# enricobottazzi/zk-fhe

Measured on AMD Instinct MI355X. Metric: BFV proofs/sec (k=13), higher is better.
Workload: dtype u32x8 (256-bit Montgomery integers over BN254 Fr/Fq)

## Files before the change

### include/zkfhe.h

```cpp
#ifndef ZKFHE_H
#define ZKFHE_H
#include <stddef.h>
#include <stdint.h>

#ifdef __cplusplus
extern "C" {
#endif

#define ZKFHE_OK 0
#define ZKFHE_EINVAL (-1)
#define ZKFHE_EHIP (-2)
#define ZKFHE_ENOMEM (-3)
#define ZKFHE_ENODEV (-4)

typedef struct zkfhe_ctx zkfhe_ctx;
typedef struct zkfhe_basis zkfhe_basis;

typedef struct { uint64_t l[4]; } zkfhe_fr;
typedef struct { uint64_t l[4]; } zkfhe_fq;
typedef struct { zkfhe_fq x, y; } zkfhe_g1_affine;
typedef struct { zkfhe_fq x, y, zz, zzz; } zkfhe_g1_xyzz;

int zkfhe_ctx_create(int device_id, void *hip_stream, zkfhe_ctx **out);
int zkfhe_ctx_destroy(zkfhe_ctx *ctx);
// ... 140 lines not shown

typedef struct zkfhe_srs zkfhe_srs;
#define ZKFHE_SRS_HALO2_UNSAFE "halo2:ParamsKZG::setup(k, ChaCha20Rng::from_seed([0u8; 32]))"
int zkfhe_srs_create(zkfhe_ctx *ctx, uint32_t k, const uint8_t *seed, size_t seed_len, zkfhe_srs **out);
int zkfhe_srs_save(zkfhe_ctx *ctx, const zkfhe_srs *srs, const char *path);
int zkfhe_srs_drop_host_copy(zkfhe_srs *srs);
int zkfhe_srs_load(zkfhe_ctx *ctx, const char *path, zkfhe_srs **out);
int zkfhe_srs_g2(const zkfhe_srs *srs, uint8_t g2_le[128], uint8_t s_g2_le[128]);
int zkfhe_srs_set_g2(zkfhe_srs *srs, const uint8_t g2_le[128], const uint8_t s_g2_le[128]);
int zkfhe_srs_file_g2(const char *path, uint32_t *k_out, uint8_t g2_le[128], uint8_t s_g2_le[128]);
int zkfhe_chacha20_block(const uint8_t key[32], const uint32_t counter_nonce[4], uint8_t out[64]);
int zkfhe_srs_from_points(zkfhe_ctx *ctx, uint32_t k, const zkfhe_g1_affine *g_host, const zkfhe_g1_affine *g_lagrange_host, zkfhe_srs **out);
int zkfhe_srs_create_sharded(zkfhe_ctx *ctx, zkfhe_comm *comm, uint32_t k, const uint8_t *seed, size_t seed_len, zkfhe_srs **out);
int zkfhe_srs_destroy(zkfhe_ctx *ctx, zkfhe_srs *srs);
int zkfhe_srs_table_bits(const zkfhe_srs *srs, int *wide_calls);
int zkfhe_srs_table_info(const zkfhe_srs *srs, int bits[2], uint64_t *bytes, int *narrowed);

typedef struct zkfhe_bfv_pk zkfhe_bfv_pk;
int zkfhe_bfv_keygen(zkfhe_ctx *ctx, const zkfhe_srs *srs, const char *input_json, const zkfhe_bfv_params *params,
                     const zkfhe_bfv_config *config, zkfhe_bfv_pk **out);
int zkfhe_bfv_pk_destroy(zkfhe_ctx *ctx, zkfhe_bfv_pk *pk);
int zkfhe_bfv_pk_release_ctx(zkfhe_ctx *ctx, zkfhe_bfv_pk *pk);
int zkfhe_bfv_pk_info(const zkfhe_bfv_pk *pk, uint8_t vk_digest[32], uint32_t *n_fixed, uint32_t *n_sigma);
int zkfhe_bfv_pk_commitments(const zkfhe_bfv_pk *pk, uint8_t *fixed_out, uint8_t *sigma_out);
int zkfhe_bfv_pk_prefix_cache(const zkfhe_bfv_pk *pk, int capacity, uint64_t *hits, uint64_t *misses, uint64_t *entries);
int zkfhe_bfv_pk_prehash(const zkfhe_bfv_pk *pk, const char *input_json, uint64_t *started, uint64_t *taken, uint64_t *pending);
int zkfhe_bfv_pk_break_points(const zkfhe_bfv_pk *pk, int which, uint32_t *out, uint32_t *count);

int zkfhe_bfv_pk_export_vk(const zkfhe_bfv_pk *pk, uint8_t *out, size_t cap, size_t *len);
int zkfhe_bfv_witness_stream(zkfhe_ctx *ctx, const zkfhe_bfv_pk *pk, const char *input_json, const uint8_t gamma_le[32], uint8_t *cells_out,
                             size_t cap_cells, size_t *n_cells);
int zkfhe_lookup_permute(zkfhe_ctx *ctx, const zkfhe_fr *cols_dev, size_t n_cols, size_t n, uint32_t usable_rows, zkfhe_fr *a_dev,
                         zkfhe_fr *s_dev, int *not_in_table);
int zkfhe_bfv_pk_save(zkfhe_ctx *ctx, const zkfhe_bfv_pk *pk, const char *path);
int zkfhe_bfv_pk_load(zkfhe_ctx *ctx, const zkfhe_srs *srs, const char *path, zkfhe_bfv_pk **out);

int zkfhe_snark_encode(const uint8_t *instances_le, size_t n_instances, const uint8_t *proof, size_t proof_len, uint8_t *out, size_t cap, size_t *len);
int zkfhe_snark_decode(const uint8_t *snark, size_t snark_len, uint8_t *instances_le, size_t *n_instances, uint8_t *proof, size_t *proof_len);

int zkfhe_bfv_verify(const uint8_t *vk_bytes, size_t vk_len, const uint8_t *instances, size_t n_instances, const uint8_t *proof,
                     size_t proof_len, const uint8_t *srs_seed, size_t seed_len, int *accepted, char *err, size_t err_len);
int zkfhe_bfv_verify_g2(const uint8_t *vk_bytes, size_t vk_len, const uint8_t *instances, size_t n_instances, const uint8_t *proof, size_t proof_len,
                        const uint8_t g2[128], const uint8_t s_g2[128], int *accepted, char *err, size_t err_len);

int zkfhe_bfv_verify_batch(zkfhe_ctx *ctx, const uint8_t *vk_bytes, size_t vk_len, size_t n_proofs, const uint8_t *const *instances,
                           const size_t *n_instances, const uint8_t *const *proofs, const size_t *proof_lens, const uint8_t *srs_seed,
                           size_t seed_len, const uint8_t *g2, const uint8_t *s_g2, int *accepted, char *errs, size_t err_stride);

int zkfhe_bfv_prove(zkfhe_ctx *ctx, const zkfhe_srs *srs, const zkfhe_bfv_pk *pk, const char *input_json,
                    const uint8_t seed[32], uint8_t *proof_out, size_t proof_cap, size_t *proof_len,
                    uint8_t *instances_out, size_t *n_instances, float *timings_ms);

typedef struct {
  const uint64_t *pk0, *pk1, *m, *u, *e0, *e1, *c0, *c1;
} zkfhe_bfv_words;
int zkfhe_bfv_prove_words(zkfhe_ctx *ctx, const zkfhe_srs *srs, const zkfhe_bfv_pk *pk, const zkfhe_bfv_words *in, const uint8_t seed[32],
                          uint8_t *proof_out, size_t proof_cap, size_t *proof_len, uint8_t *instances_out, size_t *n_instances, float *timings_ms);

int zkfhe_poly_mul_ternary_negacyclic(zkfhe_ctx *ctx, const uint64_t *a_dev, size_t a_count, const uint64_t *s_dev, size_t n_polys,
                                      uint64_t n, uint64_t q, uint64_t *out_dev, int *not_ternary);
int zkfhe_bfv_error_cdt(const zkfhe_bfv_params *params, uint64_t *thresholds, size_t *count);
int zkfhe_bfv_fhe_keypair(zkfhe_ctx *ctx, const zkfhe_bfv_params *params, const uint8_t seed[32], uint64_t *sk_out, uint64_t *pk0_out,
                          uint64_t *pk1_out);
int zkfhe_bfv_encrypt(zkfhe_ctx *ctx, const zkfhe_bfv_params *params, const uint64_t *pk0, const uint64_t *pk1, size_t n_msgs,
                      const uint64_t *m, const uint8_t seed[32], uint64_t first_index, uint64_t *u_out, uint64_t *e0_out,
                      uint64_t *e1_out, uint64_t *c0_out, uint64_t *c1_out);
// ... 73 lines not shown
```

### zk-fhe_amd/__init__.py

```python
import ctypes
import os

import numpy as np

_HERE = os.path.dirname(os.path.abspath(__file__))
LIB_PATH = os.path.join(_HERE, "libzkfhe_hip.so")
_lib = None

PROF_G1_DECOMPRESS, PROF_MSM_SEGMENTED = 3, 4
PROF_BFV_SAMPLE, PROF_RNS_NTT, PROF_RNS_EPILOGUE = 5, 6, 7
PROF_BFV_TENSOR, PROF_BFV_RELIN, PROF_BFV_EVAL_EPILOGUE, PROF_BFV_ELEMENTWISE = 8, 9, 10, 11
PROF_BFV_SHARE_SUM, PROF_BFV_DECRYPT_COMBINE = 12, 13
PROF_BFV_GALOIS, PROF_BFV_SLOT_NTT = 14, 15
PROF_BFV_HOIST, PROF_BFV_LINEAR = 16, 17

EXPORTS = [
    "zkfhe_ctx_create", "zkfhe_ctx_destroy", "zkfhe_last_error", "zkfhe_sync", "zkfhe_stream", "zkfhe_device_info",
    "zkfhe_dev_alloc", "zkfhe_dev_free", "zkfhe_upload", "zkfhe_download", "zkfhe_copy_dev", "zkfhe_memset_dev",
    "zkfhe_timer_start", "zkfhe_timer_stop_ms", "zkfhe_prof_enable", "zkfhe_prof_reset", "zkfhe_prof_read", "zkfhe_prof_read_ops", "zkfhe_ctx_last_proof_marks",
    "zkfhe_fr_add", "zkfhe_fr_sub", "zkfhe_fr_mul", "zkfhe_fr_scale", "zkfhe_fr_to_mont", "zkfhe_fr_from_mont",
    "zkfhe_fr_batch_invert", "zkfhe_fr_sqr_chain", "zkfhe_fq29_sqr_chain",
    "zkfhe_ntt_batch", "zkfhe_ntt_batch_to", "zkfhe_coset_ntt_batch",
    "zkfhe_basis_create", "zkfhe_basis_destroy", "zkfhe_basis_len", "zkfhe_msm_batch",
    "zkfhe_g1_add", "zkfhe_g1_mul", "zkfhe_msm_sparse", "zkfhe_msm_batch_xyzz", "zkfhe_msm_sparse_xyzz", "zkfhe_g1_xyzz_to_affine", "zkfhe_basis_has_multiples", "zkfhe_basis_table_bits", "zkfhe_basis_table_bytes", "zkfhe_srs_table_bits", "zkfhe_srs_table_info",
    "zkfhe_comm_unique_id", "zkfhe_comm_create", "zkfhe_comm_create_with_transport", "zkfhe_comm_destroy", "zkfhe_comm_rank", "zkfhe_comm_world", "zkfhe_comm_active",
    "zkfhe_comm_point_range", "zkfhe_comm_all_gather", "zkfhe_comm_all_gather_async", "zkfhe_msm_batch_sharded", "zkfhe_msm_batch_sharded_async", "zkfhe_comm_join", "zkfhe_comm_record_event", "zkfhe_srs_create_sharded",
    "zkfhe_witness_poly_mul_u64", "zkfhe_host_poly_mul_u32", "zkfhe_witness_div_mod",
    "zkfhe_bfv_build_tables", "zkfhe_bfv_auto_config", "zkfhe_bfv_tables_free", "zkfhe_bfv_tables_count", "zkfhe_bfv_tables_copy_advice",
    "zkfhe_bfv_tables_copy_fixed", "zkfhe_bfv_tables_copy_instance", "zkfhe_bfv_tables_copy_copies",
    "zkfhe_bfv_tables_copy_break_points", "zkfhe_bfv_mock_check", "zkfhe_bfv_tables_poke_advice",
    "zkfhe_srs_create", "zkfhe_srs_from_points", "zkfhe_srs_destroy", "zkfhe_srs_save", "zkfhe_srs_drop_host_copy", "zkfhe_srs_load", "zkfhe_srs_g2", "zkfhe_srs_set_g2", "zkfhe_srs_file_g2",
    "zkfhe_chacha20_block", "zkfhe_snark_encode", "zkfhe_snark_decode", "zkfhe_bfv_keygen", "zkfhe_bfv_pk_destroy", "zkfhe_bfv_pk_release_ctx", "zkfhe_bfv_pk_info", "zkfhe_bfv_pk_prefix_cache",
    "zkfhe_bfv_pk_commitments", "zkfhe_bfv_pk_break_points", "zkfhe_bfv_pk_prehash", "zkfhe_bfv_prove", "zkfhe_bfv_pk_export_vk", "zkfhe_bfv_pk_save", "zkfhe_bfv_pk_load", "zkfhe_bfv_witness_stream", "zkfhe_lookup_permute", "zkfhe_bfv_verify", "zkfhe_bfv_verify_g2",
    "zkfhe_g1_decompress", "zkfhe_msm_segmented", "zkfhe_bfv_verify_batch",
    "zkfhe_poly_mul_ternary_negacyclic", "zkfhe_bfv_error_cdt", "zkfhe_bfv_fhe_keypair", "zkfhe_bfv_encrypt", "zkfhe_bfv_decrypt", "zkfhe_bfv_prove_words",
    "zkfhe_bfv_add", "zkfhe_bfv_sum", "zkfhe_bfv_add_plain", "zkfhe_bfv_mul_plain", "zkfhe_bfv_relin_digits", "zkfhe_bfv_relin_keygen",
    "zkfhe_bfv_mul", "zkfhe_bfv_noise",
    "zkfhe_bfv_keygen_share", "zkfhe_bfv_share_aggregate", "zkfhe_bfv_relin_share1", "zkfhe_bfv_relin_share2", "zkfhe_bfv_decrypt_share",
    "zkfhe_bfv_decrypt_combine",
    "zkfhe_bfv_slot_count", "zkfhe_bfv_galois_element", "zkfhe_bfv_slot_sum_elements", "zkfhe_bfv_encode_slots", "zkfhe_bfv_decode_slots",
    "zkfhe_bfv_galois_keygen", "zkfhe_bfv_apply_galois", "zkfhe_bfv_slot_sum", "zkfhe_bfv_galois_share",
    "zkfhe_bfv_apply_galois_many", "zkfhe_bfv_linear_transform",
    "zkfhe_transcript_create", "zkfhe_transcript_destroy", "zkfhe_transcript_common_scalar", "zkfhe_transcript_write_scalar",
    "zkfhe_transcript_common_point", "zkfhe_transcript_write_point", "zkfhe_transcript_squeeze", "zkfhe_transcript_bytes",
    "zkfhe_poseidon_permute", "zkfhe_poseidon_constants", "zkfhe_poseidon_hash_many", "zkfhe_host_hash_mode", "zkfhe_prover_gate",
    "zkfhe_version",
]


os.environ.setdefault("GPU_MAX_HW_QUEUES", "2")


class ZkfheError(RuntimeError):
    pass


def load_library():
    global _lib
    if _lib is not None:
        return _lib
    if not os.path.exists(LIB_PATH):
        raise ZkfheError("HIP extension %s is missing: run `python zk-fhe_amd/build.py` (or __graft_entry__.build())" % LIB_PATH)
    lib = ctypes.CDLL(LIB_PATH)
    vp, sz, ci = ctypes.c_void_p, ctypes.c_size_t, ctypes.c_int
    lib.zkfhe_last_error.restype = ctypes.c_char_p
    lib.zkfhe_last_error.argtypes = [vp]
# ... 1440 lines not shown
```

### zk-fhe_amd/host/prove.hip

```cpp
#include "prover_internal.hpp"

int alloc_witness_buffers(zkfhe_ctx *ctx, const zkfhe_bfv_pk *pk, Workspace *ws) {
  if (ws->stream.p) return ZKFHE_OK;
  const size_t N = pk->prm.N;
  CK(ws->stream.alloc(ctx, (pk->gate1_cells + 8) * 32));
  CK(ws->pool.alloc(ctx, 40 * (2 * N + 8) * 32));
  CK(ws->invtmp.alloc(ctx, (pk->n_inv_slots + 8) * 32));
  ZK_HIP(ctx, hipHostMalloc((void **)&ws->host_pool, 24 * (2 * N + 8) * 32, hipHostMallocDefault));
  ws->host_poly_len = 2 * N + 8;
  ZK_HIP(ctx, hipHostMalloc((void **)&ws->host_poly, ws->host_poly_len * 32, hipHostMallocDefault));
  CK(ws->wblind.alloc(ctx, 256));
  ZK_HIP(ctx, hipHostMalloc((void **)&ws->ring, Workspace::RING_BYTES, hipHostMallocDefault));
  CK(ws->dev_ring.alloc(ctx, Workspace::RING_BYTES));
  {
    const CircuitConfig &c = pk->cfg;
    const size_t max_items = (size_t)c.n_advice() + c.n_fixed() + 2 + c.n_perm() + c.n_chunks() + 3 * c.n_lookup;
    ws->out_pts_cap = std::max<size_t>(ws->n_all, c.n_perm()) + 16;
    ws->out_ev_off = ws->out_pts_cap * PT_SLOT;
    ws->out_ev_cap = max_items * 4;
    ws->out_flag_off = ws->out_ev_off + ws->out_ev_cap * 32;
    ZK_HIP(ctx, hipHostMalloc((void **)&ws->host_out, ws->out_flag_off + 256, hipHostMallocDefault));
    memset(ws->host_out, 0, ws->out_flag_off + 256);
  }
  ZK_HIP(ctx, hipHostMalloc((void **)&ws->host_pts, ((size_t)pk->cfg.n_gate0 + 1) * PT_SLOT, hipHostMallocDefault));
// ... 433 lines not shown
  std::mutex mu;
  std::condition_variable cv;
  int slots = 0;
  uint64_t next_ticket = 0, serving = 0;
};
struct GateHold {
  bool held = false;
  void enter() { held = HeavyGate::get().enter(); }
  void leave() {
    if (held) HeavyGate::get().leave();
    held = false;
  }
  ~GateHold() { leave(); }
};

struct Trace {
  bool on;
  double t0, last, cpu_last;
  unsigned long tid;
  static double thread_cpu_ms() {
    timespec ts;
    clock_gettime(CLOCK_THREAD_CPUTIME_ID, &ts);
    return ts.tv_sec * 1e3 + ts.tv_nsec * 1e-6;
  }
  Trace() : on(getenv("ZKFHE_TRACE") != nullptr), t0(now_ms()), last(t0), cpu_last(on ? thread_cpu_ms() : 0), tid((unsigned long)std::hash<std::thread::id>()(std::this_thread::get_id()) % 10000) {}
  void mark(const char *what) {
    if (!on) return;
    const double t = now_ms(), c = thread_cpu_ms();
    fprintf(stderr, "[zkfhe trace %04lu] %8.3f ms (+%7.3f, cpu %6.3f) %s @%.3f\n", tid, t - t0, t - last, c - cpu_last, what, t);
    last = t;
    cpu_last = c;
  }
};

int prove_impl(zkfhe_ctx *ctx, const zkfhe_srs *srs, zkfhe_bfv_pk *pk, const char *input_json, const FastInput *words, const uint8_t seed[32],
               std::vector<uint8_t> &proof, std::vector<U256> &instances, float *timings) {
  const CircuitConfig &cfg = pk->cfg;
  const size_t n = cfg.n(), u = cfg.u(), ne = 4 * n;
  const unsigned k = cfg.k;
  const double t_start = now_ms();
  Trace trace;
  zkp::RngSeed rseed;
  memcpy(rseed.w, seed, 32);
  const size_t nbl_all = n - u;
  const uint64_t ctr_adv = 0, ctr_lk = (uint64_t)cfg.n_advice() * nbl_all, ctr_pz = ctr_lk + 2 * (uint64_t)cfg.n_lookup * nbl_all,
                 ctr_lz = ctr_pz + (uint64_t)cfg.n_chunks() * (nbl_all - 1), ctr_rand = ctr_lz + (uint64_t)cfg.n_lookup * (nbl_all - 1);
  auto rng_fill = [&](hipStream_t stream, uint64_t ctr0, uint64_t ctr_col_stride, Fr *dst, size_t per_col, size_t col_stride, size_t n_cols) -> int {
    if (!per_col || !n_cols) return ZKFHE_OK;
    zkp::k_rng_fill<<<grid_for(ctx, per_col * n_cols), 256, 0, stream>>>(rseed, ctr0, ctr_col_stride, dst, per_col, col_stride, n_cols);
    ZK_LAUNCH_CHECK(ctx);
    return ZKFHE_OK;
  };
  Transcript tr(cfg.transcript);
  const NttDomain *dom;
  CK(zk_domain(ctx, (int)k, &dom));
  Workspace *ws;
  CK(get_workspace(ctx, pk, &ws));
  GpuPolyMul gpu_mul(ctx, ws);
  struct BackendGuard {
    explicit BackendGuard(PolyMulBackend *b) { poly_mul_backend() = b; }
    ~BackendGuard() { poly_mul_backend() = nullptr; }
  } guard(&gpu_mul);
  const zkfhe_basis *small_basis = srs->g_lagrange_small ? srs->g_lagrange_small : srs->g_lagrange;
  CK(zkfhe_sync(ctx));
  CK(alloc_witness_buffers(ctx, pk, ws));
  ws->ring_off = ws->ring_flushed = 0;
// ... 229 lines not shown
  const Fr beta = mont(beta_c), gamma = mont(gamma_c);
  GateHold gate;
  if (!srs->sharded()) gate.enter();
  {
    if (instances.size() < ws->inst_count)
      ZK_HIP(ctx, hipMemsetAsync(ws->inst_l.fr() + instances.size(), 0, (ws->inst_count - instances.size()) * 32, ctx->stream));
    if (inst_via_ring) {
      CK(flush_staged(ctx, ws));
      if (!instances.empty()) CK(zkfhe_fr_to_mont(ctx, (const zkfhe_fr *)inst_staged, (zkfhe_fr *)ws->inst_l.p, instances.size()));
    } else {
      CK(upload_canon(ctx, ws->inst_l.fr(), instances.data(), instances.size()));
    }
    ws->inst_count = instances.size();
  }
  U256 dcan;
  memcpy(dcan.l, DELTA_CANON, 32);
  Fr *beta_delta_dev = (Fr *)ws->small.p;
  zkp::k_powers<<<1, 256, 0, ctx->stream>>>(beta, mont(dcan), beta_delta_dev, cfg.n_perm());
  ZK_LAUNCH_CHECK(ctx);
  zkp::PermArgs pa;
  pa.adv = ws->adv_l.fr();
  pa.constcol = pk->fixed_l.fr() + (size_t)cfg.fix_const() * n;
  pa.inst = ws->inst_l.fr();
  pa.sigma = pk->sigma_l.fr();
  pa.wpow = dom->fwd;
  pa.beta_delta = beta_delta_dev;
  pa.beta = beta;
  pa.gamma = gamma;
  pa.n_advice = cfg.n_advice();
  pa.n_perm = cfg.n_perm();
  pa.chunk = cfg.chunk();
  pa.n_chunks = cfg.n_chunks();
  pa.n = n;
  const size_t nch = cfg.n_chunks();
  zkp::k_perm_num_den<<<grid_for(ctx, nch * n), 256, 0, ctx->stream>>>(pa, ws->num.fr(), ws->den.fr());
  ZK_LAUNCH_CHECK(ctx);
  CK(zkfhe_fr_batch_invert(ctx, (zkfhe_fr *)ws->den.p, nch * n));
  CK(zkfhe_fr_mul(ctx, (const zkfhe_fr *)ws->num.p, (const zkfhe_fr *)ws->den.p, (zkfhe_fr *)ws->num.p, nch * n));
  Fr *totals_dev = (Fr *)ws->small.p + 4096;
  auto prefix_products = [&](const Fr *ratio, Fr *z, size_t n_cols) -> int {
    if (n <= 65536) {
      zkp::k_prefix_product<<<(unsigned)n_cols, 1024, 0, ctx->stream>>>(ratio, z, totals_dev, n, (unsigned)u);
      ZK_LAUNCH_CHECK(ctx);
      return ZKFHE_OK;
    }
    const unsigned seg_len = 32768, segs = (unsigned)(n / seg_len);
    Fr *seg = ws->den.fr();
    if ((size_t)n_cols * segs * 32 > ws->den.bytes) return zk_fail_msg(ctx, ZKFHE_EINVAL, "prefix products: segment buffer too small");
    zkp::k_prefix_seg_totals<<<dim3(segs, (unsigned)n_cols), 1024, 0, ctx->stream>>>(ratio, seg, n, (unsigned)u, seg_len);
    ZK_LAUNCH_CHECK(ctx);
    zkp::k_prefix_seg_scan<<<(unsigned)((n_cols + 63) / 64), 64, 0, ctx->stream>>>(seg, segs, (unsigned)n_cols, totals_dev);
    ZK_LAUNCH_CHECK(ctx);
    zkp::k_prefix_seg_apply<<<dim3(segs, (unsigned)n_cols), 1024, 0, ctx->stream>>>(ratio, seg, z, n, (unsigned)u, seg_len);
    ZK_LAUNCH_CHECK(ctx);
    return ZKFHE_OK;
  };
  CK(prefix_products(ws->num.fr(), ws->pz_l.fr(), nch));
  int *const closes = ws->out_flags();
  closes[0] = closes[1] = 1;
  {
    zkp::k_chunk_carry<<<1, 1024, 0, ctx->stream>>>(totals_dev, (unsigned)nch, 0, closes);
    ZK_LAUNCH_CHECK(ctx);
    zkp::k_scale_rows<<<grid_for(ctx, nch * (u + 1)), 256, 0, ctx->stream>>>(ws->pz_l.fr(), totals_dev, n, (unsigned)(u + 1), (unsigned)nch);
    ZK_LAUNCH_CHECK(ctx);
    const size_t nb = n - u - 1;
    CK(rng_fill(ctx->stream, ctr_pz, nb, ws->pz_l.fr() + (u + 1), nb, n, nch));
  }
  if (cfg.n_lookup) {
    const size_t nl = cfg.n_lookup;
    zkp::k_lookup_num_den<<<grid_for(ctx, nl * n), 256, 0, ctx->stream>>>(ws->adv_l.fr() + (size_t)cfg.adv_lookup0() * n,
                                                                          pk->fixed_l.fr() + (size_t)cfg.fix_table() * n, ws->la_l.fr(), ws->ls_l.fr(),
                                                                          beta, gamma, (unsigned)nl, n, ws->num.fr(), ws->den.fr());
    ZK_LAUNCH_CHECK(ctx);
    CK(zkfhe_fr_batch_invert(ctx, (zkfhe_fr *)ws->den.p, nl * n));
    CK(zkfhe_fr_mul(ctx, (const zkfhe_fr *)ws->num.p, (const zkfhe_fr *)ws->den.p, (zkfhe_fr *)ws->num.p, nl * n));
    CK(prefix_products(ws->num.fr(), ws->lz_l.fr(), nl));
    zkp::k_chunk_carry<<<1, 1024, 0, ctx->stream>>>(totals_dev, (unsigned)nl, 1, closes + 1);
    ZK_LAUNCH_CHECK(ctx);
    const size_t nb = n - u - 1;
    CK(rng_fill(ctx->stream, ctr_lz, nb, ws->lz_l.fr() + (u + 1), nb, n, nl));
  }
  std::vector<AffinePoint> pz_commit, lz_commit;
  CK(commit_cols_out(ctx, srs, srs->g_lagrange, ws->pz_l.fr(), nch + cfg.n_lookup, ws, pz_commit));
  if (!closes[0]) return zk_fail_msg(ctx, ZKFHE_EINVAL, "permutation argument does not close: a copy constraint is violated");
  if (!closes[1]) return zk_fail_msg(ctx, ZKFHE_EINVAL, "lookup argument does not close");
  tr.write_points(pz_commit);
  lz_commit.assign(pz_commit.begin() + nch, pz_commit.end());
  pz_commit.resize(nch);
  Fr *rand_c = ws->misc.fr() + 8 * n, *rand_l = ws->misc.fr() + 9 * n, *H_c = ws->misc.fr() + 10 * n, *H_l = ws->misc.fr() + 11 * n;
  if (early_rand) {
    ZK_HIP(ctx, hipEventSynchronize(ws->ev_rand));
    ZK_HIP(ctx, hipStreamWaitEvent(ctx->stream, ws->ev_rand, 0));
    AffinePoint rp;
    points_canon(srs, ws->host_rand_pt, 1, &rp);
    tr.write_point(rp);
  } else {
    CK(rng_fill(ctx->stream, ctr_rand, 0, rand_c, n, n, 1));
    std::vector<AffinePoint> rand_commit;
    CK(commit_cols_out(ctx, srs, srs->g, rand_c, 1, ws, rand_commit));
    tr.write_point(rand_commit[0]);
  }
  const Fr y = mont(tr.squeeze());
  const double t_commit = now_ms();
  trace.mark("grand products + commits");
  const int q_rows = pk->ext_rows;
  const unsigned W_sh = srs->sharded() ? (unsigned)zkfhe_comm_world(srs->comm) : 1u, r_sh = srs->sharded() ? (unsigned)zkfhe_comm_rank(srs->comm) : 0u;
  const size_t c_lo = nch * r_sh / W_sh, c_hi = nch * (r_sh + 1) / W_sh;
  auto owns_chunk = [&](size_t j) { return j >= c_lo && j < c_hi; };
  auto owns_col = [&](size_t perm_col) { return owns_chunk(perm_col / cfg.chunk()); };
  if (W_sh == 1) {
    CK(extend_cols(ctx, pk, ws, ws->all_l.fr(), ws->n_all, ws->all_ext.fr()));
  } else {
// ... 467 lines not shown
  ZK_ARG(ctx, srs && pk && words && seed && proof_out && proof_len);
  const uint64_t *src[8] = {words->pk0, words->pk1, words->m, words->u, words->e0, words->e1, words->c0, words->c1};
  for (const uint64_t *p : src) ZK_ARG(ctx, p != nullptr);
  try {
    pos::BulkClientScope in_flight;
    const size_t N = pk->prm.N;
    FastInput in;
    for (int k = 0; k < 8; ++k) in.a[k].assign(src[k], src[k] + N);
    in.a[8].assign(N + 1, 0);
    in.a[8][0] = in.a[8][N] = 1;
    std::vector<uint8_t> proof;
    std::vector<U256> inst;
    int rc = prove_impl(ctx, srs, const_cast<zkfhe_bfv_pk *>(pk), nullptr, &in, seed, proof, inst, timings_ms);
    if (rc) return rc;
    return copy_proof_out(ctx, proof, inst, proof_out, proof_cap, proof_len, instances_out, n_instances);
  } catch (const std::exception &e) {
    return zk_fail_msg(ctx, ZKFHE_EINVAL, e.what());
  }
}


int zkfhe_prover_gate(int n) { return HeavyGate::get().set(n); }

int zkfhe_lookup_permute(zkfhe_ctx *ctx, const zkfhe_fr *cols_dev, size_t n_cols, size_t n, uint32_t usable_rows, zkfhe_fr *a_dev, zkfhe_fr *s_dev, int *not_in_table) {
  ZK_ENTER(ctx);
  ZK_ARG(ctx, cols_dev && a_dev && s_dev && not_in_table && n_cols > 0 && n_cols < 65536 && usable_rows <= n && usable_rows >= 256);
  void *flag;
  CK(zk_scratch(ctx, 3, 64 + n_cols * 256 * sizeof(unsigned), &flag));
  ZK_HIP(ctx, hipMemsetAsync(flag, 0, 4, ctx->stream));
  CK(zkw::lookup_permute(ctx, (const Fr *)cols_dev, n, usable_rows, (unsigned)n_cols, (Fr *)a_dev, (Fr *)s_dev, (int *)flag, (unsigned *)((char *)flag + 64)));
  return zkfhe_download(ctx, not_in_table, flag, 4);
}

int zkfhe_bfv_pk_prehash(const zkfhe_bfv_pk *pk_c, const char *input_json, uint64_t *started, uint64_t *taken, uint64_t *pending) {
  if (!pk_c) return ZKFHE_EINVAL;
  zkfhe_bfv_pk *pk = const_cast<zkfhe_bfv_pk *>(pk_c);
  int rc = ZKFHE_OK;
  if (input_json) {
    const uint32_t kind = pk->cfg.transcript;
    const U256 digest = pk->vk_digest;
    const BfvParams prm = pk->prm;
    PrefixCache *cache = &pk->prefix;
    const bool ok = pk->prehash.start(input_json, strlen(input_json), [kind, digest, prm, cache](const std::string &text, std::vector<U256> &inst, Transcript::State &out) {
      struct PublicInputsKnown {};
      try {
        Context ctx0(CTX_PHASE0, false, false);
        std::vector<Cell> make_public;
        BfvState st;
        const auto on_public = [&](const std::vector<Cell> &pub) {
          inst.reserve(pub.size());
          for (const Cell &c : pub) inst.push_back(c.value);
          throw PublicInputsKnown{};
        };
        if (!bfv_phase0_fast(ctx0, text.c_str(), text.size(), prm, make_public, st, on_public))
          (void)bfv_phase0(ctx0, CircuitInput::parse_json(text.c_str()), prm, make_public, on_public);
        throw std::runtime_error("phase 0 ended without public inputs");
      } catch (const PublicInputsKnown &) {
      }
      const size_t n_key = std::min<size_t>(inst.size(), 2 * (size_t)prm.N);
      Transcript tr(kind);
      tr.common_scalar(digest);
      Transcript::State mid;
      size_t from = 0;
      if (n_key && cache->capacity()) {
        if (cache->lookup(inst.data(), n_key, mid)) {
          tr.restore(mid);
// ... 57 lines not shown
```

### zk-fhe_amd/host/prover_kernels.hip.hpp

```cpp
#pragma once
#include "../csrc/ctx.hpp"
#include "../csrc/fr29.hip.hpp"

namespace zkp {

using zk::Fr;

static __global__ void __launch_bounds__(256) k_powers(Fr start, Fr base, Fr *__restrict__ out, size_t n) {
  for (size_t i = blockIdx.x * (size_t)blockDim.x + threadIdx.x; i < n; i += (size_t)gridDim.x * blockDim.x) {
    Fr r = start, b = base;
    for (size_t e = i; e; e >>= 1) {
      if (e & 1) r = r * b;
      b = zk::fp_sqr<zk::FrP>(b);
    }
    out[i] = r;
  }
}

__device__ __forceinline__ unsigned long long rotr64(unsigned long long x, int n) { return (x >> n) | (x << (64 - n)); }
__device__ __forceinline__ Fr rng_draw(const unsigned long long seed[4], unsigned long long ctr) {
  typedef unsigned long long u64;
  const u64 IV[8] = {0x6a09e667f3bcc908ULL, 0xbb67ae8584caa73bULL, 0x3c6ef372fe94f82bULL, 0xa54ff53a5f1d36f1ULL,
                     0x510e527fade682d1ULL, 0x9b05688c2b3e6c1fULL, 0x1f83d9abfb41bd6bULL, 0x5be0cd19137e2179ULL};
  const unsigned char S[12][16] = {
// ... 134 lines not shown
  }
}

static __global__ void __launch_bounds__(1024) k_prefix_product(const Fr *__restrict__ ratio, Fr *__restrict__ z, Fr *__restrict__ total, size_t n,
                                                         unsigned u) {
  __shared__ Fr sh[1024];
  const size_t col = blockIdx.x;
  const Fr *r = ratio + col * n;
  Fr *o = z + col * n;
  const unsigned per = (unsigned)((n + 1023) / 1024);
  const unsigned lo = threadIdx.x * per;
  Fr local = Fr::one();
  for (unsigned k = 0; k < per; ++k) {
    const unsigned i = lo + k;
    if (i < u) local = local * r[i];
  }
  sh[threadIdx.x] = local;
  __syncthreads();
  for (unsigned d = 1; d < 1024; d <<= 1) {
    Fr v = sh[threadIdx.x];
    Fr other = threadIdx.x >= d ? sh[threadIdx.x - d] : Fr::one();
    __syncthreads();
    if (threadIdx.x >= d) sh[threadIdx.x] = other * v;
    __syncthreads();
  }
  Fr acc = threadIdx.x ? sh[threadIdx.x - 1] : Fr::one();
  for (unsigned k = 0; k < per; ++k) {
    const unsigned i = lo + k;
    if (i <= u) o[i] = acc;
    if (i < u) acc = acc * r[i];
  }
  if (threadIdx.x == 1023) total[col] = sh[1023];
}
static __global__ void __launch_bounds__(1024) k_prefix_seg_totals(const Fr *__restrict__ ratio, Fr *__restrict__ seg_total, size_t n, unsigned u, unsigned seg_len) {
  __shared__ Fr sh[1024];
  const size_t col = blockIdx.y;
  const unsigned seg = blockIdx.x, base = seg * seg_len;
  const Fr *r = ratio + col * n;
  const unsigned per = (seg_len + 1023) / 1024, lo = base + threadIdx.x * per;
  Fr local = Fr::one();
  for (unsigned k = 0; k < per; ++k) {
    const unsigned i = lo + k;
    if (i < u && i < base + seg_len) local = local * r[i];
  }
  sh[threadIdx.x] = local;
  __syncthreads();
  for (unsigned d = 512; d > 0; d >>= 1) {
    if (threadIdx.x < d) sh[threadIdx.x] = sh[threadIdx.x] * sh[threadIdx.x + d];
    __syncthreads();
  }
  if (threadIdx.x == 0) seg_total[col * gridDim.x + seg] = sh[0];
}
static __global__ void __launch_bounds__(64) k_prefix_seg_scan(Fr *__restrict__ seg_total, unsigned segs, unsigned n_cols, Fr *__restrict__ total) {
  const unsigned col = blockIdx.x * blockDim.x + threadIdx.x;
  if (col >= n_cols) return;
  Fr acc = Fr::one();
  for (unsigned s = 0; s < segs; ++s) {
    const Fr t = seg_total[(size_t)col * segs + s];
    seg_total[(size_t)col * segs + s] = acc;
    acc = acc * t;
  }
  total[col] = acc;
}
static __global__ void __launch_bounds__(1024) k_prefix_seg_apply(const Fr *__restrict__ ratio, const Fr *__restrict__ seg_carry, Fr *__restrict__ z, size_t n, unsigned u,
                                                            unsigned seg_len) {
  __shared__ Fr sh[1024];
// ... 334 lines not shown
```

Measured before the change: 248.6.

## Fuse permutation and lookup grand products into single segmented kernel with one inversion

Replaces the multi-kernel grand-product pipeline (num/den kernel, batch inversion, elementwise multiply, prefix product) with one fused kernel per segment. The kernel computes factors inline, scans numerator and reversed denominator products in shared memory, and needs only one field inversion per block. Columns are split into power-of-two segments sized to the CU count to raise parallelism, and the segments are stitched afterwards by the carry and scale kernels. It adds an env toggle, an A/B comparison API, and extra recomputation of factors when rows exceed the register-kept window.

Measured after the change: 248.4. About the same (-0.1%).

```diff
diff --git a/include/zkfhe.h b/include/zkfhe.h
--- a/include/zkfhe.h
+++ b/include/zkfhe.h
@@ -196,6 +196,17 @@
                              size_t cap_cells, size_t *n_cells);
 int zkfhe_lookup_permute(zkfhe_ctx *ctx, const zkfhe_fr *cols_dev, size_t n_cols, size_t n, uint32_t usable_rows, zkfhe_fr *a_dev,
                          zkfhe_fr *s_dev, int *not_in_table);
+typedef struct zkfhe_grand_product_cols {
+  const zkfhe_fr *adv, *constcol, *inst;
+  const zkfhe_fr *sigma;
+  const zkfhe_fr *wpow;
+  const zkfhe_fr *lookup_inputs, *table;
+  const zkfhe_fr *la, *ls;
+} zkfhe_grand_product_cols;
+int zkfhe_grand_products_ab(zkfhe_ctx *ctx, const zkfhe_grand_product_cols *cols, const uint8_t beta_mont[32], const uint8_t gamma_mont[32],
+                            uint32_t log_n, uint32_t usable_rows, uint32_t n_advice, uint32_t n_perm, uint32_t chunk, uint32_t n_lookup, uint32_t segs,
+                            zkfhe_fr *z_chain_dev, zkfhe_fr *totals_chain_dev, zkfhe_fr *z_fused_dev, zkfhe_fr *totals_fused_dev,
+                            int closes_chain[2], int closes_fused[2], uint32_t *segs_used);
 int zkfhe_bfv_pk_save(zkfhe_ctx *ctx, const zkfhe_bfv_pk *pk, const char *path);
 int zkfhe_bfv_pk_load(zkfhe_ctx *ctx, const zkfhe_srs *srs, const char *path, zkfhe_bfv_pk **out);
 
diff --git a/zk-fhe_amd/__init__.py b/zk-fhe_amd/__init__.py
--- a/zk-fhe_amd/__init__.py
+++ b/zk-fhe_amd/__init__.py
@@ -31,7 +31,7 @@
     "zkfhe_bfv_tables_copy_break_points", "zkfhe_bfv_mock_check", "zkfhe_bfv_tables_poke_advice",
     "zkfhe_srs_create", "zkfhe_srs_from_points", "zkfhe_srs_destroy", "zkfhe_srs_save", "zkfhe_srs_drop_host_copy", "zkfhe_srs_load", "zkfhe_srs_g2", "zkfhe_srs_set_g2", "zkfhe_srs_file_g2",
     "zkfhe_chacha20_block", "zkfhe_snark_encode", "zkfhe_snark_decode", "zkfhe_bfv_keygen", "zkfhe_bfv_pk_destroy", "zkfhe_bfv_pk_release_ctx", "zkfhe_bfv_pk_info", "zkfhe_bfv_pk_prefix_cache",
-    "zkfhe_bfv_pk_commitments", "zkfhe_bfv_pk_break_points", "zkfhe_bfv_pk_prehash", "zkfhe_bfv_prove", "zkfhe_bfv_pk_export_vk", "zkfhe_bfv_pk_save", "zkfhe_bfv_pk_load", "zkfhe_bfv_witness_stream", "zkfhe_lookup_permute", "zkfhe_bfv_verify", "zkfhe_bfv_verify_g2",
+    "zkfhe_bfv_pk_commitments", "zkfhe_bfv_pk_break_points", "zkfhe_bfv_pk_prehash", "zkfhe_bfv_prove", "zkfhe_bfv_pk_export_vk", "zkfhe_bfv_pk_save", "zkfhe_bfv_pk_load", "zkfhe_bfv_witness_stream", "zkfhe_lookup_permute", "zkfhe_grand_products_ab", "zkfhe_bfv_verify", "zkfhe_bfv_verify_g2",
     "zkfhe_g1_decompress", "zkfhe_msm_segmented", "zkfhe_bfv_verify_batch",
     "zkfhe_poly_mul_ternary_negacyclic", "zkfhe_bfv_error_cdt", "zkfhe_bfv_fhe_keypair", "zkfhe_bfv_encrypt", "zkfhe_bfv_decrypt", "zkfhe_bfv_prove_words",
     "zkfhe_bfv_add", "zkfhe_bfv_sum", "zkfhe_bfv_add_plain", "zkfhe_bfv_mul_plain", "zkfhe_bfv_relin_digits", "zkfhe_bfv_relin_keygen",
diff --git a/zk-fhe_amd/host/prove.hip b/zk-fhe_amd/host/prove.hip
--- a/zk-fhe_amd/host/prove.hip
+++ b/zk-fhe_amd/host/prove.hip
@@ -489,6 +489,73 @@
     cpu_last = c;
   }
 };
+
+unsigned grand_product_segs(zkfhe_ctx *ctx, size_t n, size_t nch, size_t nl) {
+  unsigned s = 1;
+  while (2 * s * nch + nl <= (size_t)ctx->num_cu && 2 * s * nch + nl <= 4096 && n / (2 * s) >= 2048) s *= 2;
+  return s;
+}
+int launch_grand_products(zkfhe_ctx *ctx, const zkp::GrandArgs &ga, unsigned n_lookup) {
+  const unsigned blocks = ga.p.n_chunks * ga.segs + n_lookup;
+  if (!blocks) return ZKFHE_OK;
+  if (ga.p.n > 65536 || ga.u >= ga.p.n || !ga.segs || (ga.segs & (ga.segs - 1)) || ga.p.n % ga.segs)
+    return zk_fail_msg(ctx, ZKFHE_EINVAL, "fused grand products: rows or segments out of range");
+  const size_t rows = n_lookup ? ga.p.n : ga.p.n / ga.segs;
+  if (rows <= 8192) zkp::k_grand_product_fused<true><<<blocks, 1024, 0, ctx->stream>>>(ga);
+  else zkp::k_grand_product_fused<false><<<blocks, 1024, 0, ctx->stream>>>(ga);
+  ZK_LAUNCH_CHECK(ctx);
+  return ZKFHE_OK;
+}
+int chain_grand_products(zkfhe_ctx *ctx, Fr *z, Fr *totals, size_t n, size_t u, size_t nch, unsigned segs, size_t nl, int *closes) {
+  const size_t blocks = nch * segs, rows = segs > 1 ? n / segs : u + 1, stride = n / segs;
+  if (blocks) {
+    zkp::k_chunk_carry<<<1, 1024, 0, ctx->stream>>>(totals, (unsigned)blocks, 0, closes);
+    ZK_LAUNCH_CHECK(ctx);
+    zkp::k_scale_rows<<<grid_for(ctx, blocks * rows), 256, 0, ctx->stream>>>(z, totals, stride, (unsigned)rows, (unsigned)blocks);
+    ZK_LAUNCH_CHECK(ctx);
+  }
+  if (nl) {
+    zkp::k_chunk_carry<<<1, 1024, 0, ctx->stream>>>(totals + blocks, (unsigned)nl, 1, closes + 1);
+    ZK_LAUNCH_CHECK(ctx);
+  }
+  return ZKFHE_OK;
+}
+int grand_products_chain(zkfhe_ctx *ctx, const zkp::PermArgs &pa, const Fr *a_cols, const Fr *table, const Fr *la, const Fr *ls, unsigned n_lookup, unsigned u,
+                         Fr *num, Fr *den, size_t den_bytes, Fr *z, Fr *totals_dev) {
+  const size_t n = pa.n, nch = pa.n_chunks, nl = n_lookup;
+  auto prefix_products = [&](const Fr *ratio, Fr *zc, Fr *tot, size_t n_cols) -> int {
+    if (n <= 65536) {
+      zkp::k_prefix_product<<<(unsigned)n_cols, 1024, 0, ctx->stream>>>(ratio, zc, tot, n, u);
+      ZK_LAUNCH_CHECK(ctx);
+      return ZKFHE_OK;
+    }
+    const unsigned seg_len = 32768, segs = (unsigned)(n / seg_len);
+    Fr *seg = den;
+    if ((size_t)n_cols * segs * 32 > den_bytes) return zk_fail_msg(ctx, ZKFHE_EINVAL, "prefix products: segment buffer too small");
+    zkp::k_prefix_seg_totals<<<dim3(segs, (unsigned)n_cols), 1024, 0, ctx->stream>>>(ratio, seg, n, u, seg_len);
+    ZK_LAUNCH_CHECK(ctx);
+    zkp::k_prefix_seg_scan<<<(unsigned)((n_cols + 63) / 64), 64, 0, ctx->stream>>>(seg, segs, (unsigned)n_cols, tot);
+    ZK_LAUNCH_CHECK(ctx);
+    zkp::k_prefix_seg_apply<<<dim3(segs, (unsigned)n_cols), 1024, 0, ctx->stream>>>(ratio, seg, zc, n, u, seg_len);
+    ZK_LAUNCH_CHECK(ctx);
+    return ZKFHE_OK;
+  };
+  if (nch) {
+    zkp::k_perm_num_den<<<grid_for(ctx, nch * n), 256, 0, ctx->stream>>>(pa, num, den);
+    ZK_LAUNCH_CHECK(ctx);
+    CK(zkfhe_fr_batch_invert(ctx, (zkfhe_fr *)den, nch * n));
+    CK(zkfhe_fr_mul(ctx, (const zkfhe_fr *)num, (const zkfhe_fr *)den, (zkfhe_fr *)num, nch * n));
+    CK(prefix_products(num, z, totals_dev, nch));
+  }
+  if (nl) {
+    zkp::k_lookup_num_den<<<grid_for(ctx, nl * n), 256, 0, ctx->stream>>>(a_cols, table, la, ls, pa.beta, pa.gamma, (unsigned)nl, n, num, den);
+    ZK_LAUNCH_CHECK(ctx);
+    CK(zkfhe_fr_batch_invert(ctx, (zkfhe_fr *)den, nl * n));
+    CK(zkfhe_fr_mul(ctx, (const zkfhe_fr *)num, (const zkfhe_fr *)den, (zkfhe_fr *)num, nl * n));
+    CK(prefix_products(num, z + nch * n, totals_dev + nch, nl));
+  }
+  return ZKFHE_OK;
+}
 
 int prove_impl(zkfhe_ctx *ctx, const zkfhe_srs *srs, zkfhe_bfv_pk *pk, const char *input_json, const FastInput *words, const uint8_t seed[32],
                std::vector<uint8_t> &proof, std::vector<U256> &instances, float *timings) {
@@ -784,52 +851,33 @@
   pa.chunk = cfg.chunk();
   pa.n_chunks = cfg.n_chunks();
   pa.n = n;
-  const size_t nch = cfg.n_chunks();
-  zkp::k_perm_num_den<<<grid_for(ctx, nch * n), 256, 0, ctx->stream>>>(pa, ws->num.fr(), ws->den.fr());
-  ZK_LAUNCH_CHECK(ctx);
-  CK(zkfhe_fr_batch_invert(ctx, (zkfhe_fr *)ws->den.p, nch * n));
-  CK(zkfhe_fr_mul(ctx, (const zkfhe_fr *)ws->num.p, (const zkfhe_fr *)ws->den.p, (zkfhe_fr *)ws->num.p, nch * n));
+  const size_t nch = cfg.n_chunks(), nl = cfg.n_lookup;
   Fr *totals_dev = (Fr *)ws->small.p + 4096;
-  auto prefix_products = [&](const Fr *ratio, Fr *z, size_t n_cols) -> int {
-    if (n <= 65536) {
-      zkp::k_prefix_product<<<(unsigned)n_cols, 1024, 0, ctx->stream>>>(ratio, z, totals_dev, n, (unsigned)u);
-      ZK_LAUNCH_CHECK(ctx);
-      return ZKFHE_OK;
-    }
-    const unsigned seg_len = 32768, segs = (unsigned)(n / seg_len);
-    Fr *seg = ws->den.fr();
-    if ((size_t)n_cols * segs * 32 > ws->den.bytes) return zk_fail_msg(ctx, ZKFHE_EINVAL, "prefix products: segment buffer too small");
-    zkp::k_prefix_seg_totals<<<dim3(segs, (unsigned)n_cols), 1024, 0, ctx->stream>>>(ratio, seg, n, (unsigned)u, seg_len);
-    ZK_LAUNCH_CHECK(ctx);
-    zkp::k_prefix_seg_scan<<<(unsigned)((n_cols + 63) / 64), 64, 0, ctx->stream>>>(seg, segs, (unsigned)n_cols, totals_dev);
-    ZK_LAUNCH_CHECK(ctx);
-    zkp::k_prefix_seg_apply<<<dim3(segs, (unsigned)n_cols), 1024, 0, ctx->stream>>>(ratio, seg, z, n, (unsigned)u, seg_len);
-    ZK_LAUNCH_CHECK(ctx);
-    return ZKFHE_OK;
-  };
-  CK(prefix_products(ws->num.fr(), ws->pz_l.fr(), nch));
   int *const closes = ws->out_flags();
   closes[0] = closes[1] = 1;
+  const char *fused_env = getenv("ZKFHE_FUSED_PRODUCTS");
+  const bool fused = n <= 65536 && !(fused_env && fused_env[0] == '0');
+  const unsigned segs = fused ? grand_product_segs(ctx, n, nch, nl) : 1;
+  if (fused) {
+    zkp::GrandArgs ga;
+    ga.p = pa;
+    ga.a_cols = ws->adv_l.fr() + (size_t)cfg.adv_lookup0() * n;
+    ga.table = pk->fixed_l.fr() + (size_t)cfg.fix_table() * n;
+    ga.la = ws->la_l.fr();
+    ga.ls = ws->ls_l.fr();
+    ga.z = ws->pz_l.fr();
+    ga.total = totals_dev;
+    ga.u = (unsigned)u;
+    ga.segs = segs;
+    CK(launch_grand_products(ctx, ga, (unsigned)nl));
+  } else {
+    CK(grand_products_chain(ctx, pa, ws->adv_l.fr() + (size_t)cfg.adv_lookup0() * n, pk->fixed_l.fr() + (size_t)cfg.fix_table() * n, ws->la_l.fr(),
+                            ws->ls_l.fr(), (unsigned)nl, (unsigned)u, ws->num.fr(), ws->den.fr(), ws->den.bytes, ws->pz_l.fr(), totals_dev));
+  }
+  CK(chain_grand_products(ctx, ws->pz_l.fr(), totals_dev, n, u, nch, segs, nl, closes));
   {
-    zkp::k_chunk_carry<<<1, 1024, 0, ctx->stream>>>(totals_dev, (unsigned)nch, 0, closes);
-    ZK_LAUNCH_CHECK(ctx);
-    zkp::k_scale_rows<<<grid_for(ctx, nch * (u + 1)), 256, 0, ctx->stream>>>(ws->pz_l.fr(), totals_dev, n, (unsigned)(u + 1), (unsigned)nch);
-    ZK_LAUNCH_CHECK(ctx);
     const size_t nb = n - u - 1;
     CK(rng_fill(ctx->stream, ctr_pz, nb, ws->pz_l.fr() + (u + 1), nb, n, nch));
-  }
-  if (cfg.n_lookup) {
-    const size_t nl = cfg.n_lookup;
-    zkp::k_lookup_num_den<<<grid_for(ctx, nl * n), 256, 0, ctx->stream>>>(ws->adv_l.fr() + (size_t)cfg.adv_lookup0() * n,
-                                                                          pk->fixed_l.fr() + (size_t)cfg.fix_table() * n, ws->la_l.fr(), ws->ls_l.fr(),
-                                                                          beta, gamma, (unsigned)nl, n, ws->num.fr(), ws->den.fr());
-    ZK_LAUNCH_CHECK(ctx);
-    CK(zkfhe_fr_batch_invert(ctx, (zkfhe_fr *)ws->den.p, nl * n));
-    CK(zkfhe_fr_mul(ctx, (const zkfhe_fr *)ws->num.p, (const zkfhe_fr *)ws->den.p, (zkfhe_fr *)ws->num.p, nl * n));
-    CK(prefix_products(ws->num.fr(), ws->lz_l.fr(), nl));
-    zkp::k_chunk_carry<<<1, 1024, 0, ctx->stream>>>(totals_dev, (unsigned)nl, 1, closes + 1);
-    ZK_LAUNCH_CHECK(ctx);
-    const size_t nb = n - u - 1;
     CK(rng_fill(ctx->stream, ctr_lz, nb, ws->lz_l.fr() + (u + 1), nb, n, nl));
   }
   std::vector<AffinePoint> pz_commit, lz_commit;
@@ -1363,6 +1411,65 @@
   return zkfhe_download(ctx, not_in_table, flag, 4);
 }
 
+int zkfhe_grand_products_ab(zkfhe_ctx *ctx, const zkfhe_grand_product_cols *c, const uint8_t beta_mont[32], const uint8_t gamma_mont[32], uint32_t log_n,
+                            uint32_t usable_rows, uint32_t n_advice, uint32_t n_perm, uint32_t chunk, uint32_t n_lookup, uint32_t segs, zkfhe_fr *z_chain_dev,
+                            zkfhe_fr *totals_chain_dev, zkfhe_fr *z_fused_dev, zkfhe_fr *totals_fused_dev, int closes_chain[2], int closes_fused[2],
+                            uint32_t *segs_used) {
+  ZK_ENTER(ctx);
+  ZK_ARG(ctx, c && beta_mont && gamma_mont && z_chain_dev && totals_chain_dev && z_fused_dev && totals_fused_dev && closes_chain && closes_fused);
+  ZK_ARG(ctx, log_n >= 1 && log_n <= 16 && usable_rows < (1u << log_n) && chunk >= 1 && n_perm >= 1 && n_perm <= n_advice + 2 && n_perm <= 4096 && n_lookup <= 1024);
+  ZK_ARG(ctx, c->adv && c->constcol && c->inst && c->sigma && c->wpow && (!n_lookup || (c->lookup_inputs && c->table && c->la && c->ls)));
+  const size_t n = (size_t)1 << log_n, nch = (n_perm + chunk - 1) / chunk;
+  if (!segs) segs = grand_product_segs(ctx, n, nch, n_lookup);
+  ZK_ARG(ctx, !(segs & (segs - 1)) && segs <= n && nch * segs + n_lookup <= 4096);
+  if (segs_used) *segs_used = segs;
+  void *scr;
+  const size_t head = ((size_t)n_perm + nch * segs + n_lookup) * 32 + 64, arr = std::max<size_t>(nch, n_lookup) * n * 32;
+  CK(zk_scratch(ctx, 3, head + 2 * arr, &scr));
+  Fr *beta_delta = (Fr *)scr, *carry = beta_delta + n_perm;
+  int *flags = (int *)(carry + nch * segs + n_lookup);
+  Fr *num = (Fr *)((char *)scr + head), *den = (Fr *)((char *)scr + head + arr);
+  zkp::PermArgs pa;
+  memcpy(&pa.beta, beta_mont, 32);
+  memcpy(&pa.gamma, gamma_mont, 32);
+  U256 dcan;
+  memcpy(dcan.l, DELTA_CANON, 32);
+  zkp::k_powers<<<1, 256, 0, ctx->stream>>>(pa.beta, mont(dcan), beta_delta, n_perm);
+  ZK_LAUNCH_CHECK(ctx);
+  pa.adv = (const Fr *)c->adv;
+  pa.constcol = (const Fr *)c->constcol;
+  pa.inst = (const Fr *)c->inst;
+  pa.sigma = (const Fr *)c->sigma;
+  pa.wpow = (const Fr *)c->wpow;
+  pa.beta_delta = beta_delta;
+  pa.n_advice = n_advice;
+  pa.n_perm = n_perm;
+  pa.chunk = chunk;
+  pa.n_chunks = (unsigned)nch;
+  pa.n = n;
+  auto finish = [&](zkfhe_fr *z, const zkfhe_fr *totals, unsigned sg, int out[2]) -> int {
+    ZK_HIP(ctx, hipMemcpyAsync(carry, totals, (nch * sg + n_lookup) * 32, hipMemcpyDeviceToDevice, ctx->stream));
+    ZK_HIP(ctx, hipMemsetAsync(flags, 0xff, 8, ctx->stream));
+    CK(chain_grand_products(ctx, (Fr *)z, carry, n, usable_rows, nch, sg, n_lookup, flags));
+    return zkfhe_download(ctx, out, flags, 8);
+  };
+  CK(grand_products_chain(ctx, pa, (const Fr *)c->lookup_inputs, (const Fr *)c->table, (const Fr *)c->la, (const Fr *)c->ls, n_lookup, usable_rows, num, den, arr,
+                          (Fr *)z_chain_dev, (Fr *)totals_chain_dev));
+  CK(finish(z_chain_dev, totals_chain_dev, 1, closes_chain));
+  zkp::GrandArgs ga;
+  ga.p = pa;
+  ga.a_cols = (const Fr *)c->lookup_inputs;
+  ga.table = (const Fr *)c->table;
+  ga.la = (const Fr *)c->la;
+  ga.ls = (const Fr *)c->ls;
+  ga.z = (Fr *)z_fused_dev;
+  ga.total = (Fr *)totals_fused_dev;
+  ga.u = usable_rows;
+  ga.segs = segs;
+  CK(launch_grand_products(ctx, ga, n_lookup));
+  return finish(z_fused_dev, totals_fused_dev, segs, closes_fused);
+}
+
 int zkfhe_bfv_pk_prehash(const zkfhe_bfv_pk *pk_c, const char *input_json, uint64_t *started, uint64_t *taken, uint64_t *pending) {
   if (!pk_c) return ZKFHE_EINVAL;
   zkfhe_bfv_pk *pk = const_cast<zkfhe_bfv_pk *>(pk_c);
diff --git a/zk-fhe_amd/host/prover_kernels.hip.hpp b/zk-fhe_amd/host/prover_kernels.hip.hpp
--- a/zk-fhe_amd/host/prover_kernels.hip.hpp
+++ b/zk-fhe_amd/host/prover_kernels.hip.hpp
@@ -190,6 +190,122 @@
   }
   if (threadIdx.x == 1023) total[col] = sh[1023];
 }
+struct GrandArgs {
+  PermArgs p;
+  const Fr *a_cols, *table, *la, *ls;
+  Fr *z, *total;
+  unsigned u, segs;
+};
+template <bool NUM>
+__device__ __forceinline__ Fr grand_factor(const GrandArgs &g, bool perm, unsigned lcol, unsigned i) {
+  const PermArgs &a = g.p;
+  if (!perm) {
+    const size_t at = (size_t)lcol * a.n + i;
+    return NUM ? (g.a_cols[at] + a.beta) * (g.table[i] + a.gamma) : (g.la[at] + a.beta) * (g.ls[at] + a.gamma);
+  }
+  const unsigned c0 = lcol * a.chunk, c1 = min(c0 + a.chunk, a.n_perm);
+  Fr w, r;
+  if (NUM) w = a.wpow[i];
+  for (unsigned c = c0; c < c1; ++c) {
+    const Fr v = perm_col(a, c)[i];
+    const Fr f = NUM ? v + a.beta_delta[c] * w + a.gamma : v + a.beta * a.sigma[(size_t)c * a.n + i] + a.gamma;
+    r = c == c0 ? f : r * f;
+  }
+  return r;
+}
+template <bool KEEP>
+static __global__ void __launch_bounds__(1024) k_grand_product_fused(GrandArgs g) {
+  __shared__ Fr shn[1024], shd[1024];
+  const unsigned t = threadIdx.x, n_seg_blocks = g.p.n_chunks * g.segs;
+  const bool perm = blockIdx.x < n_seg_blocks;
+  const unsigned lcol = perm ? blockIdx.x / g.segs : blockIdx.x - n_seg_blocks;
+  const unsigned n = (unsigned)g.p.n, seg_len = perm ? n / g.segs : n, base = perm ? (blockIdx.x % g.segs) * seg_len : 0u;
+  Fr *o = g.z + (size_t)(perm ? lcol : g.p.n_chunks + lcol) * n;
+  const unsigned per = (seg_len + 1023) / 1024, lo = base + t * per, u = g.u;
+  const unsigned stop = min(min(lo + per, base + seg_len), u);
+  const unsigned cnt = lo >= stop ? 0u : stop - lo;
+  Fr nu[KEEP ? 8 : 1];
+  unsigned long long zero_rows = 0;
+  Fr N = Fr::one(), S = Fr::one();
+  auto down = [&](unsigned k) {
+    const unsigned i = lo + k;
+    Fr de = grand_factor<false>(g, perm, lcol, i), x = grand_factor<true>(g, perm, lcol, i);
+    if (de.is_zero()) {
+      de = Fr::one();
+      x = Fr::zero();
+      zero_rows |= 1ull << k;
+    }
+    S = S * de;
+    o[i] = S;
+    N = N * x;
+    if constexpr (KEEP) nu[k & 7] = x;
+  };
+  if (KEEP) {
+#pragma unroll
+    for (int k = 7; k >= 0; --k)
+      if ((unsigned)k < cnt) down((unsigned)k);
+  } else {
+    for (unsigned k = cnt; k-- > 0;) down(k);
+  }
+  shn[t] = N;
+  shd[1023 - t] = S;
+  unsigned off = 1;
+  for (unsigned d = 512; d > 0; d >>= 1, off <<= 1) {
+    __syncthreads();
+    if (t < d) {
+      const unsigned ai = off * (2 * t + 1) - 1, bi = off * (2 * t + 2) - 1;
+      shn[bi] = shn[ai] * shn[bi];
+      shd[bi] = shd[ai] * shd[bi];
+    }
+  }
+  __syncthreads();
+  Fr all_n, all_d;
+  if (t == 0) {
+    all_n = shn[1023];
+    all_d = shd[1023];
+    shn[1023] = shd[1023] = Fr::one();
+  }
+  for (unsigned d = 1; d < 1024; d <<= 1) {
+    off >>= 1;
+    __syncthreads();
+    if (t < d) {
+      const unsigned ai = off * (2 * t + 1) - 1, bi = off * (2 * t + 2) - 1;
+      const Fr ln = shn[ai], ld = shd[ai], rn = shn[bi], rd = shd[bi];
+      shn[ai] = rn;
+      shd[ai] = rd;
+      shn[bi] = ln * rn;
+      shd[bi] = ld * rd;
+    }
+  }
+  __syncthreads();
+  const Fr before = shn[t], after = shd[1023 - t];
+  __syncthreads();
+  if (t == 0) {
+    const Fr inv = zk::fp_inv<zk::FrP>(all_d);
+    g.total[blockIdx.x] = all_n * inv;
+    shd[0] = inv;
+  }
+  __syncthreads();
+  const Fr dinv = shd[0];
+  Fr acc = before * dinv * after;
+  auto up = [&](unsigned k) {
+    const unsigned i = lo + k;
+    Fr x;
+    if constexpr (KEEP) x = nu[k & 7];
+    else x = (zero_rows >> k) & 1 ? Fr::zero() : grand_factor<true>(g, perm, lcol, i);
+    o[i] = acc * o[i];
+    acc = acc * x;
+  };
+  if (KEEP) {
+#pragma unroll
+    for (int k = 0; k < 8; ++k)
+      if ((unsigned)k < cnt) up((unsigned)k);
+  } else {
+    for (unsigned k = 0; k < cnt; ++k) up(k);
+  }
+  if (lo + cnt == u && lo + cnt < min(lo + per, base + seg_len)) o[u] = acc;
+}
+
 static __global__ void __launch_bounds__(1024) k_prefix_seg_totals(const Fr *__restrict__ ratio, Fr *__restrict__ seg_total, size_t n, unsigned u, unsigned seg_len) {
   __shared__ Fr sh[1024];
   const size_t col = blockIdx.y;
```
